# cohensbw/ElPhDynamics

Hardware: AMD Instinct MI355X
Metric: cg_matvecs_per_sec (higher is better)
Workload: dtype f64; 1 GPU; BASELINE config C: Holstein square L=16 Ntau=160 (N=256, Ltau=160, Ndim=40960), un-preconditioned CG iteration, 288 right-hand sides per step on each GPU = 144 independent Markov chain(s) x 2 solve(s) each (2 = the two pseudofermion solves of one HMC force evaluation), 1 GPU(s) with their own chains; nrhs=288, chains_per_gpu=144, ndim=40960, preconditioned=False, form=workgroup-resident: K iterations of the whole batch in one launch (k_cg_wg), parallelism=gpus1xchains144

## Files before the change

elphdynamics_amd/csrc/cg_wg.hip:

```cpp

#include <algorithm>
#include <atomic>
#include <type_traits>

#include "cg_fast_common.h"

#include "cg_wg_dev.h"
#include "pgrid_dev.h"

namespace wg {

#ifdef ELPH_WG_ARRIVE
__device__ unsigned long long g_wg_arrive[4096 * 4];
__device__ unsigned long long g_wg_timeline[4096 * 4];
#define TL(k) do { if (threadIdx.x == 0 && blockIdx.x < 4096) g_wg_timeline[blockIdx.x * 4 + (k)] = (unsigned long long)wall_clock64(); } while (0)
#else
#define TL(k) do { } while (0)
#endif

struct WgRankArgs { CgBufs B; ModelDev m; WgCtl R; ShardCtl Sh; };
template <int NPL, int T, bool SSH, bool UNI, int FORM, bool SHARD, bool X0Z = false, bool RANKS = false>
__global__ void __launch_bounds__(512) k_cg_wg(CgBufs B, ModelDev m, WgCtl R, ShardCtl Sh) {
    static_assert(!RANKS || SHARD, "several ranks per launch: sharded solves only");
    unsigned bid = 0;
// ... 86 lines not shown
            if (lwok) rl[j * HSL + lr + q * LSL] = rg[(size_t)(t0 + j) * N + sc[q]];
            if (X_GLB) {}
            else if (X_REG) xr[X_REG ? j : 0][q] = X0Z ? 0.0 : xg[(size_t)(t0 + j) * N + sc[q]];
            else if (lwok) xl[j * HSL + lr + q * LSL] = X0Z ? 0.0 : xg[(size_t)(t0 + j) * N + sc[q]];
        }
#pragma unroll
    for (int j = 0; j < T + 2; ++j)
#pragma unroll
        for (int q = 0; q < NPL; ++q) {
            p[j][q] = rg[(size_t)wrap(t0 + j - 1) * N + sc[q]];
            if (PH_LDS && (j == 0 || j == T + 1) && lwok) PHALO(j, q) = p[j][q];
        }
#pragma unroll
    for (int j = 0; j < NEJ; ++j)
#pragma unroll
        for (int q = 0; q < NPL; ++q) {
            const double ev = Ech[(size_t)wrap(t0 + j) * m.E_tau_stride + sc[q]];
            if (E_LDS) { if (lwok) el[j * HSL + lr + q * LSL] = ev; }
            else E[E_LDS ? 0 : j][q] = ev;
        }
    unsigned ij[NE];
    Tab<NE, UNI> tab[NT];
    SqCtx<UNI> X;
    SqSsh<NSREG, S_LDS> XS;
    HcCtx XH;
    S8Ctx X8;
    GridCtx XG;
    HgCtx XHG;
    pgrid::Ctx XT;
    if constexpr (GR) {
        XG = grid_ctx(lane, GGX, GGY, m.c_uni, m.s_uni);
        if constexpr (TG) { XT = pgrid::Tri<2, 2>::make_ctx(lane, 2 * GGX, m.c_uni, m.s_uni); XG.k4 = XT.ks; }
    } else if constexpr (HG) {
        XHG = hgrid_ctx<NPL>(lane, HLX, HLY, m.c_uni, m.s_uni);
    } else if constexpr (S8) {
        X8.th = m.s_uni / m.c_uni; X8.k4 = (m.c_uni * m.c_uni) * (m.c_uni * m.c_uni);
        X8.yx = sq_patch_ycross(lane); X8.xodd = (lane >> 1) & 1;
    } else if constexpr (HC) {
        XH.th = m.s_uni / m.c_uni; XH.k3 = m.c_uni * m.c_uni * m.c_uni;
        XH.up = (lane + 16) & (WAVE - 1); XH.dn = (lane + 48) & (WAVE - 1);
    } else if constexpr (SQ && SSH) {
        ssh_chain_select(m, rhs);
        XS.yx = sq_patch_ycross(lane);
        XS.l0 = eall + (size_t)wv * SQ_TABS * WAVE + lane;
#pragma unroll
        for (int j = 0; j <= T; ++j) {
            const double *cj = m.c + (size_t)wrap(t0 + j) * m.cs_tau_stride, *sj = m.s + (size_t)wrap(t0 + j) * m.cs_tau_stride;
            SqTabS tb;
#pragma unroll
            for (int pr = 0; pr < 2; ++pr) {
                const int b0 = m.sq_bond[0 * N + sc[2 * pr]], b2 = m.sq_bond[2 * N + sc[pr]];
                tb.ci[0][pr] = cj[b0]; tb.si[0][pr] = sj[b0];
                tb.ci[1][pr] = cj[b2]; tb.si[1][pr] = sj[b2];
            }
#pragma unroll
            for (int k = 0; k < 4; ++k) {
                const int b1 = m.sq_bond[1 * N + sc[k]], b3 = m.sq_bond[3 * N + sc[k]];
                tb.cx[0][k] = cj[b1]; tb.sx[0][k] = sj[b1];
                tb.cx[1][k] = cj[b3]; tb.sx[1][k] = sj[b3];
            }
            if (S_LDS && j == 0) {
                double *d = eall + (size_t)wv * SQ_TABS * WAVE + lane;
#pragma unroll
                for (int pr = 0; pr < 2; ++pr) {
                    d[(0 + pr) * WAVE] = tb.ci[0][pr]; d[(2 + pr) * WAVE] = tb.si[0][pr];
                    d[(4 + pr) * WAVE] = tb.ci[1][pr]; d[(6 + pr) * WAVE] = tb.si[1][pr];
                }
#pragma unroll
                for (int k = 0; k < 4; ++k) {
                    d[(8 + k) * WAVE] = tb.cx[0][k]; d[(12 + k) * WAVE] = tb.sx[0][k];
                    d[(16 + k) * WAVE] = tb.cx[1][k]; d[(20 + k) * WAVE] = tb.sx[1][k];
                }
            } else {
                XS.t[S_LDS ? (j > 0 ? j - 1 : 0) : (j < NSREG ? j : 0)] = tb;
            }
        }
    } else if constexpr (SQ) {
        X.yx = sq_patch_ycross(lane);
        if constexpr (UNI) {
            X.c[0][0] = m.c_uni; X.s[0][0] = m.s_uni / m.c_uni; X.k4 = (m.c_uni * m.c_uni) * (m.c_uni * m.c_uni);
        } else {
            X.k4 = 1.0;
#pragma unroll
            for (int col = 0; col < 4; ++col)
#pragma unroll
                for (int k = 0; k < 4; ++k) {
                    const int bd = m.sq_bond[col * N + sc[k]];
                    X.c[UNI ? 0 : col][UNI ? 0 : k] = m.c[bd];
                    X.s[UNI ? 0 : col][UNI ? 0 : k] = m.s[bd];
                }
        }
    } else {
#pragma unroll
        for (int e = 0; e < NE; ++e) ij[e] = m.lp_ij[e * WAVE + lane];
        if (SSH) {
            ssh_chain_select(m, rhs);
#pragma unroll
            for (int j = 0; j < NT; ++j)
                load_tab<NE, UNI>(tab[j], m.lp_c + (size_t)wrap(t0 + j) * m.lp_tau_stride, m.lp_s + (size_t)wrap(t0 + j) * m.lp_tau_stride, lane, m);
        } else {
            load_tab<NE, UNI>(tab[0], m.lp_c, m.lp_s, lane, m);
        }
    }
#define EXPV(j, q) (E_LDS ? el[(j) * HSL + lr + (q) * LSL] : E[(SSH || E_LDS) ? 0 : (j)][q])

    constexpr size_t SLOTS_RHS = SLOTS_PER_RHS;
    u64 *const slots0 = R.slots + (size_t)rhs * 2 * SLOTS_RHS;
    u64 *const bnd0 = R.bnd + (size_t)rhs * 2 * G * 2 * HS * 2;
    const int gm = (g == 0) ? G - 1 : g - 1, gp = (g == G - 1) ? 0 : g + 1;
    double rho = S.rho, kmin = S.kmin, eps = S.eps;
    double eps0 = S.eps0, normb = S.normb;

    if (threadIdx.x == 0) { tot[5] = 1.0; if (SHARD) bc[2] = 1.0; }
    if (G > 1) {
        if (wv == 0) {
#pragma unroll
            for (int q = 0; q < NPL; ++q) if (lwok) rhalo[lr + q * LSL] = p[0][q];
        }
        if (wv == W - 1) {
#pragma unroll
            for (int q = 0; q < NPL; ++q) if (lwok) rhalo[HSL + lr + q * LSL] = p[T + 1][q];
        }
    }
    const u64 *gaddr[NPL];
    if constexpr (SHARD) {
#pragma unroll
        for (int q = 0; q < NPL; ++q) {
            const int s = ss[q];
            gaddr[q] = (s < Sh.own_lo) ? sh_ghost(Sh.mail[Sh.rank], 0, L, Sh.cap_ghost, t0, s)
                     : (s >= Sh.own_hi && s < N) ? sh_ghost(Sh.mail[Sh.rank], 1, L, Sh.cap_ghost, t0, s - Sh.own_hi) : nullptr;
        }
        double a0 = 0.0;
#pragma unroll
        for (int q = 0; q < NPL; ++q) if (own[q]) a0 += p[1][q] * p[1][q];
        a0 = wave_sum_dpp(a0);
        if (lane == 0) partA[wv] = a0;
        wg_barrier();
        if (wv == 0) {
            const double mine = wg_sum(partA, W, lane);
            sh_publish<RANKS>(Sh, 0, g, G, mine, 1u, lane);
            const u64 *none[NPL];
#pragma unroll
            for (int q = 0; q < NPL; ++q) none[q] = nullptr;
            double tot = 0.0, dummy[NPL];
            const bool ok = sh_poll<NPL, RANKS>(Sh, true, 0, G, none, 1u, lane, R, tot, dummy);
            if (lane == 0) { bc[0] = tot; if (!ok) bc[2] = 0.0; }
        }
        wg_barrier();
        if (bc[2] == 0.0) return;
        const double bb = bc[0];
        normb = sqrt(bb); eps0 = 1.0; eps = 1.0; rho = bb; kmin = 0.0;
        wg_barrier();
    }
    const double rr_far = (P.tol * normb) * (P.tol * normb) * 1.000001, y_num = 4.0 * (eps0 * normb) * (eps0 * normb);
    const double it_kappa = 0.17 * sqrt(P.kmax);
    STAMP_DECL;
    for (long long seq = 0;; ++seq) {
        const unsigned epoch = R.epoch0 + (unsigned)seq + (SHARD ? 2u : 1u);
        const unsigned par = epoch & 1u;
        u64 *const slotsA = slots0 + (size_t)par * SLOTS_RHS, *const slotsB = slotsA + SLOTS_A;
        u64 *const bnd = bnd0 + (size_t)par * G * 2 * HS * 2;
        const size_t ghp = SHARD ? (size_t)par * 2 * L * Sh.cap_ghost * 2 : 0;
        STAMP(9);
        if (seq == 0) TL(0);
        if (seq == 1) TL(1);
        double (&w)[T + 1][NPL] = zw;
        if constexpr (S8) {
#pragma unroll
            for (int k = 0; k <= T; ++k) w[k][0] = EXPV(k, 0) * p[k][0];
            s8_sweepN<T + 1, false>(w, X8);
#pragma unroll
            for (int k = 0; k <= T; ++k) w[k][0] = p[k + 1][0] - sgn(wrap(t0 + k)) * X8.k4 * w[k][0];
            double gq[T][1];
#pragma unroll
            for (int i = 0; i < T; ++i) gq[i][0] = w[i + 1][0];
            s8_sweepN<T, true>(gq, X8);
#pragma unroll
            for (int i = 0; i < T; ++i) w[i][0] = w[i][0] - sgn(wrap(t0 + i + 1)) * X8.k4 * (EXPV(i + 1, 0) * gq[i][0]);
        } else if constexpr (HC) {
#pragma unroll
            for (int k = 0; k <= T; ++k)
#pragma unroll
                for (int q = 0; q < NPL; ++q) w[k][q] = EXPV(k, q) * ((PH_LDS && k == 0) ? PHALO(0, q) : p[k][q]);
            hc_sweepN<T + 1, false>(w, XH);
#pragma unroll
            for (int k = 0; k <= T; ++k) {
                const double sg = sgn(wrap(t0 + k)) * XH.k3;
#pragma unroll
                for (int q = 0; q < NPL; ++q) w[k][q] = ((PH_LDS && k == T) ? PHALO(1, q) : p[k + 1][q]) - sg * w[k][q];
            }
            auto rev = [&](auto nb, auto j0c) __attribute__((always_inline)) {
                constexpr int NB = decltype(nb)::value, j0 = decltype(j0c)::value;
                double gq[NB][NPL];
#pragma unroll
                for (int i = 0; i < NB; ++i)
#pragma unroll
                    for (int q = 0; q < NPL; ++q) gq[i][q] = w[j0 + i + 1][q];
                hc_sweepN<NB, true>(gq, XH);
#pragma unroll
                for (int i = 0; i < NB; ++i) {
                    const double sg = sgn(wrap(t0 + j0 + i + 1)) * XH.k3;
#pragma unroll
                    for (int q = 0; q < NPL; ++q) w[j0 + i][q] = w[j0 + i][q] - sg * (EXPV(j0 + i + 1, q) * gq[i][q]);
                }
            };
            using std::integral_constant;
            if constexpr (T == 3) { rev(integral_constant<int, 2>(), integral_constant<int, 0>()); rev(integral_constant<int, 1>(), integral_constant<int, 2>()); }
            else rev(integral_constant<int, T>(), integral_constant<int, 0>());
        } else if constexpr (HG) {
#pragma unroll
            for (int k = 0; k <= T; ++k)
#pragma unroll
                for (int q = 0; q < NPL; ++q) w[k][q] = EXPV(k, q) * p[k][q];
            hgrid_sweepN<NPL, T + 1, false>(w, XHG);
#pragma unroll
            for (int k = 0; k <= T; ++k) {
                const double sg = sgn(wrap(t0 + k)) * XHG.k3;
#pragma unroll
                for (int q = 0; q < NPL; ++q) w[k][q] = p[k + 1][q] - sg * w[k][q];
            }
            double gq[T][NPL];
#pragma unroll
            for (int i = 0; i < T; ++i)
#pragma unroll
                for (int q = 0; q < NPL; ++q) gq[i][q] = w[i + 1][q];
            hgrid_sweepN<NPL, T, true>(gq, XHG);
#pragma unroll
            for (int i = 0; i < T; ++i) {
                const double sg = sgn(wrap(t0 + i + 1)) * XHG.k3;
#pragma unroll
                for (int q = 0; q < NPL; ++q) w[i][q] = w[i][q] - sg * (EXPV(i + 1, q) * gq[i][q]);
            }
        } else if constexpr (GR) {
#pragma unroll
            for (int k = 0; k <= T; ++k)
#pragma unroll
                for (int q = 0; q < 4; ++q) w[k][q] = EXPV(k, q) * p[k][q];
            if constexpr (TG) {
#pragma unroll
                for (int k = 0; k <= T; ++k) pgrid::Tri<2, 2>::apply<false>(w[k], XT);
            } else grid_sweepN<T + 1, false, (T >= 4) ? 1 : 2>(w, XG);
#pragma unroll
            for (int k = 0; k <= T; ++k) {
                const double sg = sgn(wrap(t0 + k)) * XG.k4;
#pragma unroll
                for (int q = 0; q < 4; ++q) w[k][q] = p[k + 1][q] - sg * w[k][q];
            }
            constexpr int RBG = (T >= 4) ? 2 : T;
#pragma unroll
            for (int j0 = 0; j0 < T; j0 += RBG) {
                double gq[RBG][4];
#pragma unroll
                for (int i = 0; i < RBG; ++i)
#pragma unroll
                    for (int q = 0; q < 4; ++q) gq[i][q] = w[j0 + i + 1][q];
                if constexpr (TG) {
#pragma unroll
                    for (int i = 0; i < RBG; ++i) pgrid::Tri<2, 2>::apply<true>(gq[i], XT);
                } else grid_sweepN<RBG, true, (T >= 4) ? 1 : 2>(gq, XG);
#pragma unroll
                for (int i = 0; i < RBG; ++i) {
                    const double sg = sgn(wrap(t0 + j0 + i + 1)) * XG.k4;
#pragma unroll
                    for (int q = 0; q < 4; ++q) w[j0 + i][q] = w[j0 + i][q] - sg * (EXPV(j0 + i + 1, q) * gq[i][q]);
                }
            }
        } else if constexpr (SQ) {
#pragma unroll
            for (int k = 0; k <= T; ++k)
#pragma unroll
                for (int q = 0; q < 4; ++q) w[k][q] = EXPV(k, q) * p[k][q];
            if constexpr (SSH) sq_sweepS<T + 1, false, 0>(w, XS);
            else sq_sweepN<T + 1, false, UNI>(w, X);
#pragma unroll
            for (int k = 0; k <= T; ++k) {
                const double sg = UNI ? sgn(wrap(t0 + k)) * X.k4 : sgn(wrap(t0 + k));
#pragma unroll
                for (int q = 0; q < 4; ++q) w[k][q] = p[k + 1][q] - sg * w[k][q];
            }
            constexpr int RB = (T >= 4) ? 2 : T;
#pragma unroll
            for (int j0 = 0; j0 < T; j0 += RB) {
                double gq[RB][4];
#pragma unroll
                for (int i = 0; i < RB; ++i)
#pragma unroll
                    for (int q = 0; q < 4; ++q) gq[i][q] = w[j0 + i + 1][q];
                if constexpr (SSH) sq_sweepS<RB, true, 1>(gq, XS);
                else sq_sweepN<RB, true, UNI>(gq, X);
#pragma unroll
                for (int i = 0; i < RB; ++i) {
                    const double sg = UNI ? sgn(wrap(t0 + j0 + i + 1)) * X.k4 : sgn(wrap(t0 + j0 + i + 1));
#pragma unroll
                    for (int q = 0; q < 4; ++q) w[j0 + i][q] = w[j0 + i][q] - sg * (EXPV(j0 + i + 1, q) * gq[i][q]);
                }
            }
        } else {
#pragma unroll
            for (int k = 0; k <= T; ++k)
#pragma unroll
                for (int q = 0; q < NPL; ++q) slab[k * SL + lane + q * WAVE] = EXPV(k, q) * p[k][q];
            WAVE_LDS_ORDER();
            sweepN<NPL, T + 1, false, UNI, NT, SSH ? 1 : 0, 0>(slab, ij, tab, m.ncol);
#pragma unroll
            for (int k = 0; k <= T; ++k) {
                const double sg = sgn(wrap(t0 + k));
#pragma unroll
                for (int q = 0; q < NPL; ++q) w[k][q] = p[k + 1][q] - sg * slab[k * SL + lane + q * WAVE];
            }
            WAVE_LDS_ORDER();
#pragma unroll
            for (int j = 0; j < T; ++j)
#pragma unroll
                for (int q = 0; q < NPL; ++q) slab[j * SL + lane + q * WAVE] = w[j + 1][q];
            WAVE_LDS_ORDER();
            sweepN<NPL, T, true, UNI, NT, SSH ? 1 : 0, SSH ? 1 : 0>(slab, ij, tab, m.ncol);
#pragma unroll
            for (int j = 0; j < T; ++j) {
                const double sg = sgn(wrap(t0 + j + 1));
#pragma unroll
                for (int q = 0; q < NPL; ++q) w[j][q] = w[j][q] - sg * EXPV(j + 1, q) * slab[j * SL + lane + q * WAVE];
            }
            WAVE_LDS_ORDER();
        }
        double (&z)[T + 1][NPL] = zw;
        int lane_b = lane;
        if constexpr (HC && T >= 3) asm volatile("" : "+v"(lane_b));
        double rr;
        {
        double s_pz = 0.0, s_rz = 0.0, s_zz = 0.0, s_rr = 0.0;
#pragma unroll
        for (int j = 0; j < T; ++j)
#pragma unroll
            for (int q = 0; q < NPL; ++q)
                if (own[q]) {
                    const double rv = rl[j * HSL + lr + q * LSL];
                    s_pz += p[j + 1][q] * z[j][q];
                    s_rz += rv * z[j][q];
                    s_zz += z[j][q] * z[j][q];
                    s_rr += rv * rv;
                }
        {
            const double k4 = wave_sum4(s_pz, s_rz, s_zz, s_rr, lane);
            if (lane < 4) part[lane * 8 + wv] = k4;
        }
        if constexpr (X_GLB) {
#pragma unroll
            for (int j = 0; j < T; ++j)
#pragma unroll
                for (int q = 0; q < NPL; ++q) xr[X_REG ? j : 0][q] = xg[(size_t)(t0 + j) * N + sc[q]];
        }
        if constexpr (SHARD) {
            const int prev = (Sh.rank + Sh.P - 1) % Sh.P, next = (Sh.rank + 1) % Sh.P;
#pragma unroll
            for (int q = 0; q < NPL; ++q) {
                const int s = ss[q];
                const u64 bits = (u64)__double_as_longlong(z[0][q]), tag = (u64)epoch << 32;
                if (s >= Sh.own_lo && s < Sh.own_lo + Sh.n_to_prev) {
                    u64 *d = sh_ghost(Sh.mail[prev], 1, L, Sh.cap_ghost, t0, s - Sh.own_lo) + ghp;
                    st_mail<RANKS>(d, tag | (bits & 0xFFFFFFFFull)); st_mail<RANKS>(d + 1, tag | (bits >> 32));
                }
                if (s >= Sh.own_hi - Sh.n_to_next && s < Sh.own_hi) {
                    u64 *d = sh_ghost(Sh.mail[next], 0, L, Sh.cap_ghost, t0, s - (Sh.own_hi - Sh.n_to_next)) + ghp;
                    st_mail<RANKS>(d, tag | (bits & 0xFFFFFFFFull)); st_mail<RANKS>(d + 1, tag | (bits >> 32));
                }
            }
        }
        if (G > 1) {
            if (wv == 0) {
#pragma unroll
                for (int q = 0; q < NPL; ++q) {
                    st_f64_gran(bnd + (((size_t)g * 2 + 0) * HS + lane_b + q * WAVE) * 2, z[0][q], epoch);
                    if constexpr (HC && T >= 3) __builtin_amdgcn_sched_barrier(0);
                }
            }
            if (wv == W - 1) {
#pragma unroll
                for (int q = 0; q < NPL; ++q) {
                    st_f64_gran(bnd + (((size_t)g * 2 + 1) * HS + lane_b + q * WAVE) * 2, z[T - 1][q], epoch);
                    if constexpr (HC && T >= 3) __builtin_amdgcn_sched_barrier(0);
                }
            }
        }
        STAMP(0);
        wg_barrier();
        STAMP(2);
        double pap, rz, zz, rr0;
        double gz[NPL];
        if constexpr (SHARD) {
            const int rw = (W >= 3) ? 1 : 0;
            u64 *rankrec = Sh.mail[Sh.rank] + (size_t)SH_MAXREC * 2 + (size_t)par * 8 * REC4;
            bool ok = true;
            if (wv == rw) publish_rec4(slotsA, g, sum_part4(part, W, lane), epoch, lane);
            {
                const bool bw = G > 1 && (wv == 0 || wv == W - 1);
                const int th = (wv == 0) ? wrap(t0 - 1) : wrap(t0 + T);
                const u64 *bh = bw ? ((wv == 0) ? bnd + (((size_t)gm * 2 + 1) * HS) * 2 : bnd + (((size_t)gp * 2 + 0) * HS) * 2) : nullptr;
                const u64 *ga2[NPL];
#pragma unroll
                for (int q = 0; q < NPL; ++q) {
                    const int s = ss[q];
                    ga2[q] = !bw ? nullptr
                           : (s < Sh.own_lo) ? sh_ghost(Sh.mail[Sh.rank], 0, L, Sh.cap_ghost, th, s) + ghp
                           : (s >= Sh.own_hi && s < N) ? sh_ghost(Sh.mail[Sh.rank], 1, L, Sh.cap_ghost, th, s - Sh.own_hi) + ghp : nullptr;
                }
                u64 a0[NPL], a1[NPL], h0[NPL], h1[NPL], c0[NPL], c1[NPL];
                long long t_start = 0;
                for (int spin = 0;; ++spin) {
                    bool good = true;
#pragma unroll
                    for (int q = 0; q < NPL; ++q) {
                        if (gaddr[q]) { a0[q] = ld_mail<RANKS>(gaddr[q] + ghp); a1[q] = ld_mail<RANKS>(gaddr[q] + ghp + 1); }
                        if (bh) { h0[q] = ld_gran(bh + 2 * (lane + q * WAVE)); h1[q] = ld_gran(bh + 2 * (lane + q * WAVE) + 1); }
                        if (ga2[q]) { c0[q] = ld_mail<RANKS>(ga2[q]); c1[q] = ld_mail<RANKS>(ga2[q] + 1); }
                    }
#pragma unroll
                    for (int q = 0; q < NPL; ++q) {
                        if (gaddr[q]) good = good && (unsigned)(a0[q] >> 32) == epoch && (unsigned)(a1[q] >> 32) == epoch;
                        if (bh) good = good && (unsigned)(h0[q] >> 32) == epoch && (unsigned)(h1[q] >> 32) == epoch;
                        if (ga2[q]) good = good && (unsigned)(c0[q] >> 32) == epoch && (unsigned)(c1[q] >> 32) == epoch;
                    }
                    if (__all(good)) break;
                    if (poll_bail<NPL>(spin, t_start, lane, R)) { ok = false; break; }
                    __builtin_amdgcn_s_sleep(1);
                }
#pragma unroll
                for (int q = 0; q < NPL; ++q) {
                    gz[q] = gaddr[q] ? __hiloint2double((int)(unsigned)a1[q], (int)(unsigned)a0[q]) : 0.0;
                    if (bw) {
                        const double hv = ga2[q] ? __hiloint2double((int)(unsigned)c1[q], (int)(unsigned)c0[q])
                                                 : __hiloint2double((int)(unsigned)h1[q], (int)(unsigned)h0[q]);
                        zhalo[((wv == 0) ? 0 : HSL) + lr + q * LSL] = hv;
                    }
                }
            }
            if (wv == rw) {
                if (g == 0) {
                    double d0, d1, t4 = 0.0;
                    if (G <= 8) { u64 v[1] = {0}; ok = poll_rec4<1>(slotsA, G, nullptr, nullptr, epoch, lane, R, v, d0, d1) && ok; t4 = sum_rec4<1>(v, G, lane); }
                    else        { u64 v[4] = {0, 0, 0, 0}; ok = poll_rec4<4>(slotsA, G, nullptr, nullptr, epoch, lane, R, v, d0, d1) && ok; t4 = sum_rec4<4>(v, G, lane); }
                    const double mine = __shfl(t4, lane & 6, WAVE);
                    if (lane < 8 * Sh.P) {
                        const u64 bits = (u64)__double_as_longlong(mine);
                        st_mail<RANKS>(Sh.mail[lane >> 3] + (size_t)SH_MAXREC * 2 + (size_t)par * 8 * REC4 + (size_t)Sh.rank * REC4 + (lane & 7),
                               ((u64)epoch << 32) | ((lane & 1) ? (bits >> 32) : (bits & 0xFFFFFFFFull)));
                    }
                }
                u64 v[1] = {0};
                long long t_start = 0;
                for (int spin = 0;; ++spin) {
                    bool good = true;
                    if (lane < REC4 * Sh.P) { v[0] = ld_mail<RANKS>(rankrec + lane); good = (unsigned)(v[0] >> 32) == epoch; }
                    if (__all(good)) break;
                    if (poll_bail<1>(spin, t_start, lane, R)) { ok = false; break; }
                    __builtin_amdgcn_s_sleep(1);
                }
                const double t4 = sum_rec4<1>(v, Sh.P, lane);
                if (lane < 8 && !(lane & 1)) tot[lane >> 1] = t4;
            }
            if (!ok && lane == 0) tot[5] = 0.0;
            wg_barrier();
            if (tot[5] == 0.0) return;
            pap = tot[0]; rz = tot[1]; zz = tot[2]; rr0 = tot[3];
        } else if (G == 1) {
            const double t4 = sum_part4(part, W, lane);
            pap = readlane_f64(t4, 0); rz = readlane_f64(t4, 8); zz = readlane_f64(t4, 16); rr0 = readlane_f64(t4, 24);
        } else {
            constexpr int NSEG = 2 * NPL;
            const int rw = (W > NSEG) ? NSEG : ((W >= 3) ? 1 : 0);
            bool ok = true;
            double t4 = 0.0;
            if (wv == rw) publish_rec4(slotsA, g, sum_part4(part, W, lane), epoch, lane);
            for (int s0 = wv; s0 < NSEG || (s0 == wv && wv == rw); s0 += 2 * W) {
                const int s1 = s0 + W;
                const u64 *b0 = nullptr, *b1 = nullptr;
                if (s0 < NSEG) b0 = bnd + ((((s0 < NPL) ? (size_t)gm * 2 + 1 : (size_t)gp * 2 + 0) * HS) + lane_b + (size_t)(s0 % NPL) * WAVE) * 2;
                if (s1 < NSEG) b1 = bnd + ((((s1 < NPL) ? (size_t)gm * 2 + 1 : (size_t)gp * 2 + 0) * HS) + lane_b + (size_t)(s1 % NPL) * WAVE) * 2;
                const bool recs = (wv == rw && s0 == wv);
                double z0 = 0.0, z1 = 0.0;
                if (G <= 8) {
                    u64 v[1] = {0};
                    ok = poll_rec4<1>(recs ? slotsA : nullptr, G, b0, b1, epoch, lane, R, v, z0, z1) && ok;
                    if (recs) t4 = sum_rec4<1>(v, G, lane);
                } else {
                    u64 v[4] = {0, 0, 0, 0};
                    ok = poll_rec4<4>(recs ? slotsA : nullptr, G, b0, b1, epoch, lane, R, v, z0, z1) && ok;
                    if (recs) t4 = sum_rec4<4>(v, G, lane);
                }
                if (b0 && lwok) zhalo[(size_t)s0 * LSL + lr] = z0;
                if (b1 && lwok) zhalo[(size_t)s1 * LSL + lr] = z1;
                if (!ok) break;
            }
            if (wv == rw && lane < 8 && !(lane & 1)) tot[lane >> 1] = t4;
            if (!ok && lane == 0) tot[5] = 0.0;
#ifdef ELPH_WG_ARRIVE
            if (!ok && lane == 0 && blockIdx.x < 4096) g_wg_arrive[blockIdx.x * 4 + 3] = ((unsigned long long)(seq + 1) << 8) | (1ull << wv);
#endif
            wg_barrier();
            if (tot[5] == 0.0) return;
            pap = tot[0]; rz = tot[1]; zz = tot[2]; rr0 = tot[3];
        }
        STAMP(1);
        rho = rr0;
        const double alpha = rr0 / pap;
        rr = rr0 + alpha * (alpha * zz - 2.0 * rz);
#pragma unroll
        for (int j = 0; j < T; ++j)
#pragma unroll
            for (int q = 0; q < NPL; ++q) {
                const double zq = (SHARD && gaddr[q]) ? gz[q] : z[j][q];
                const double rn = rl[j * HSL + lr + q * LSL] - alpha * zq;
                if (lwok) rl[j * HSL + lr + q * LSL] = rn;
                if (X_GLB) { if (lwok) xg[(size_t)(t0 + j) * N + sc[q]] = xr[X_REG ? j : 0][q] + alpha * p[j + 1][q]; }
                else if (X_REG) xr[X_REG ? j : 0][q] += alpha * p[j + 1][q];
                else if (lwok) xl[j * HSL + lr + q * LSL] += alpha * p[j + 1][q];
            }
        if (G > 1 && (wv == 0 || wv == W - 1)) {
            double *rh = rhalo + ((wv == 0) ? 0 : HSL);
            const double *zh = zhalo + ((wv == 0) ? 0 : HSL);
#pragma unroll
            for (int q = 0; q < NPL; ++q) if (lwok) rh[lr + q * LSL] = rh[lr + q * LSL] - alpha * zh[lr + q * LSL];
        }
        STAMP(3);
        if (!(rr > 1e-3 * rr0)) {
            double a = 0.0;
#pragma unroll
            for (int j = 0; j < T; ++j)
#pragma unroll
                for (int q = 0; q < NPL; ++q) if (own[q]) { const double rn = rl[j * HSL + lr + q * LSL]; a += rn * rn; }
            a = wave_sum_dpp(a);
            if (lane == 0) partF[wv] = a;
            wg_barrier();
            if constexpr (SHARD) {
                if (wv == 0) {
                    sh_publish<RANKS>(Sh, 0, g, G, wg_sum(partF, W, lane), epoch, lane);
                    const u64 *none[NPL];
#pragma unroll
                    for (int q = 0; q < NPL; ++q) none[q] = nullptr;
                    double t = 0.0, dummy[NPL];
                    const bool ok = sh_poll<NPL, RANKS>(Sh, true, 0, G, none, epoch, lane, R, t, dummy);
                    if (lane == 0) { tot[4] = t; if (!ok) tot[5] = 0.0; }
                }
                wg_barrier();
                if (tot[5] == 0.0) return;
                rr = tot[4];
            } else if (G == 1) {
                rr = wg_sum(partF, W, lane);
            } else {
                if (wv == 0) {
                    const double mine = wg_sum(partF, W, lane);
                    if (lane < 2) {
                        const u64 bits = (u64)__double_as_longlong(mine);
                        st_gran(slotsB + 2 * g + lane, ((u64)epoch << 32) | (lane ? (bits >> 32) : (bits & 0xFFFFFFFFull)));
                    }
                    u64 v = 0;
                    const bool ok = poll_records(slotsB, G, epoch, lane, R, v);
                    const int half = (int)(unsigned)v;
                    double t = 0.0;
                    for (int k = 0; k < G; ++k)
                        t += __hiloint2double(__builtin_amdgcn_readlane(half, 2 * k + 1), __builtin_amdgcn_readlane(half, 2 * k));
                    if (lane == 0) { tot[4] = t; if (!ok) tot[5] = 0.0; }
                }
                wg_barrier();
                if (tot[5] == 0.0) return;
                rr = tot[4];
            }
        }
        wg_barrier();
        STAMP(4);
        }
        STAMP(5);
        STAMP(6);
        const long long it = seq + 1;
        const bool fixed = R.fixed_iters > 0;
        int done = 0;
        const bool screened = !P.record_hist && it < (fixed ? R.fixed_iters : P.maxiter) && (fixed || rr > rr_far) &&
                              (rr + rr <= y_num || rr >= y_num + y_num) && (double)it < it_kappa;
        if (!screened) {
            eps = sqrt(rr) / normb;
            const double qq = 2.0 * (double)it / log(2.0 * eps0 / eps);
            const double val = qq * qq;
            kmin = (val > kmin) ? val : kmin;
            if (eps < P.tol) done = 1;
            else if (kmin > P.kmax) done = 2;
            else if (it >= P.maxiter) done = 3;
            if (fixed) done = (it >= R.fixed_iters) ? 3 : 0;
            if (g == 0 && wv == 0 && lane == 0 && P.record_hist) B.hist[(size_t)rhs * P.hist_stride + it] = eps;
        }
        STAMP(7);
        if (done) {
            STAMP_OUT(it);
            TL(2);
            int lane2 = lane;
            asm volatile("" : "+v"(lane2));
#pragma unroll
            for (int j = 0; j < T; ++j)
#pragma unroll
                for (int q = 0; q < NPL; ++q) {
                    const int s2 = SQ ? sq_patch_site(lane2, q) : (HC ? hc_site(lane2, q) : (S8 ? s8_site(lane2) : (GR ? grid_site(lane2, q, GGX, GGY) : (HG ? hgrid_site<NPL>(lane2, q, HLX, HLY) : lane2 + q * WAVE))));
                    if (HC ? hc_real(lane2) : (GR ? lane2 < GGX * GGY : (HG ? lane2 < (HLX / HgDim<NPL>::PX) * (HLY / HgDim<NPL>::PY) : (SQ || s2 < N)))) {
                        if (SHARD) rg[(size_t)(t0 + j) * N + s2] = rl[j * HSL + lr + q * LSL];
                        if (!X_GLB) xg[(size_t)(t0 + j) * N + s2] = X_REG ? xr[X_REG ? j : 0][q] : xl[j * HSL + lr + q * LSL];
                    }
                }
            if (g == 0 && wv == 0 && lane == 0) {
                CgState o = S;
                o.rho = rho; o.kmin = kmin; o.eps = eps; o.seq = it + 1; o.iters = it; o.done = done;
                st2[0] = o;
                st2[1] = o;
            }
            TL(3);
            return;
        }
        const double beta = rr / rho;
        rho = rr;
        {
            const bool lx = (G > 1 && wv == 0), rx = (G > 1 && wv == W - 1);
            const double *sl = rall + ((size_t)((wv > 0) ? wv - 1 : W - 1) * T + (T - 1)) * HSL;
            const double *sr = rall + ((size_t)((wv < W - 1) ? wv + 1 : 0) * T + 0) * HSL;
#pragma unroll
            for (int q = 0; q < NPL; ++q) {
                const double hl = lx ? rhalo[lr + q * LSL] : sl[lr + q * LSL];
                const double hr = rx ? rhalo[HSL + lr + q * LSL] : sr[lr + q * LSL];
                if constexpr (PH_LDS) {
                    const double n0 = hl + beta * PHALO(0, q), n1 = hr + beta * PHALO(1, q);
                    if (lwok) { PHALO(0, q) = n0; PHALO(1, q) = n1; }
                } else {
                    p[0][q] = hl + beta * p[0][q];
                    p[T + 1][q] = hr + beta * p[T + 1][q];
                }
            }
        }
#pragma unroll
        for (int j = 0; j < T; ++j)
#pragma unroll
            for (int q = 0; q < NPL; ++q) p[j + 1][q] = rl[j * HSL + lr + q * LSL] + beta * p[j + 1][q];
        STAMP(8);
    }
#undef EXPV
#undef PHALO
}


struct Shape { int T, W, G; size_t shm; bool sq, hc, s8, gr, hg; int npl; bool tg = false; };

static bool wg_no_dpp() {
    const char *e = getenv("ELPH_WG_NO_DPP");
    return e && e[0] == '1';
}

static bool sq_form(const elph_handle_s *h, const ModelDev &m) {
    return h->shape.dpp() == 2 && m.sq_bond && !wg_no_dpp();
}

static bool hc_form(const elph_handle_s *h, const ModelDev &m) {
    return h->kind == ELPH_MODEL_HOLSTEIN && h->shape.hc12() && m.uniform && !wg_no_dpp();
}

static bool s8_form(const elph_handle_s *h, const ModelDev &m) {
    return h->kind == ELPH_MODEL_HOLSTEIN && h->shape.dpp() == 1 && m.uniform && !wg_no_dpp();
}

static bool gr_form(const elph_handle_s *h, const ModelDev &m, bool for_shard = false) {
    if (h->kind != ELPH_MODEL_HOLSTEIN || !h->shape.small_square() || !m.uniform || m.grid_GX * m.grid_GY < 1 || m.grid_GX * m.grid_GY > 64 || wg_no_dpp()) return false;
    return for_shard || h->shape.dpp() == 0;
}

static bool tg_form(const elph_handle_s *h, const ModelDev &m) {
    return h->kind == ELPH_MODEL_HOLSTEIN && h->shape.kind == LatticeShape::TRIANGULAR && h->shape.GX > 0 && m.uniform && !wg_no_dpp();
}

static int hg_form(const elph_handle_s *h, const ModelDev &m, bool for_shard = false) {
    if (h->kind != ELPH_MODEL_HOLSTEIN || (h->shape.hc12() && !for_shard) || !m.uniform || wg_no_dpp()) return 0;
    return h->shape.hgrid_regs();
}

static int largest_divisor_le8(int n, int cap = 8) { for (int w = std::min(cap, n); w >= 1; --w) if (n % w == 0) return w; return 1; }

static bool pick_shape(const elph_handle_s *h, const ModelDev &m, int forceT, int nrhs, Shape *out) {
    const int L = (int)h->L;
    const bool ssh = (h->kind == ELPH_MODEL_SSH), sq = sq_form(h, m), hc = !sq && hc_form(h, m), s8 = !sq && !hc && s8_form(h, m);
    const bool tg = !sq && !hc && !s8 && tg_form(h, m);
    const bool gr = !sq && !hc && !s8 && (tg || gr_form(h, m));
    const int hgn = (!sq && !hc && !s8 && !gr) ? hg_form(h, m) : 0;
    const bool hg = hgn > 0;
    const int npl = hc ? HC_NPL : (gr ? 4 : (hg ? hgn : h->npl));
    if (h->lp_mc != 4 && !tg) return false;
    if (!hc && !gr && !hg && h->npl > 5) return false;
    bool big_batch = true;
    if (!forceT && L % 2 == 0) {
        const int G2 = (L / 2) / largest_divisor_le8(L / 2);
        big_batch = G2 <= 32 && nrhs > 8 * (32 / G2);
    }
    if (!ssh && !sq && !hc && !gr && !hg && h->npl == 1 && (big_batch || s8)) {
        const int one[3] = {4, 5, 8};
        for (int T : one) {
            if ((forceT && T != forceT) || L % T || L / T > 8 || L / T < 2) continue;
            const int W = L / T;
            const size_t SL = (size_t)npl * WAVE + 2 * WAVE, HS = (size_t)npl * WAVE;
            const size_t shm = ((size_t)W * (s8 ? 0 : T + 1) * SL + 2 * (size_t)W * T * HS + 48 + 4 * HS) * sizeof(double);
            if (shm > 160 * 1024) continue;
            out->T = T; out->W = W; out->G = 1; out->shm = shm; out->sq = false; out->hc = false; out->s8 = s8; out->gr = false; out->hg = false; out->npl = npl;
            return true;
        }
    }
    const int cand[4] = {4, 3, 2, 1};
    for (int T : cand) {
        if (forceT && T != forceT) continue;
        if (T == 3) {
            if (!hc || L % 3 || L % 2) continue;
            if (forceT != 3) {
                const int G2 = (L / 2) / largest_divisor_le8(L / 2), G3 = (L / 3) / largest_divisor_le8(L / 3);
                if (G2 > 32 || G3 > 32) continue;
                const int r2 = 8 * (32 / G2), r3 = 8 * (32 / G3);
                if (nrhs <= r2 || 8.6 * ((nrhs + r3 - 1) / r3) >= 5.7 * ((nrhs + r2 - 1) / r2)) continue;
            }
        }
        if (T == 4) {
            if (!(sq || gr) || !m.uniform || ssh) continue;
            if (forceT != 4) {
                if (L % 2) continue;
                const int G2 = (L / 2) / largest_divisor_le8(L / 2);
                if (G2 > 32 || nrhs <= 8 * (32 / G2)) continue;
            }
        }
        if (gr && T == 3) continue;
        if (hg && T > 2) continue;
        if (T == 2 && (sq || hc || gr || hg) && forceT != 2) {
            const int G1 = L / largest_divisor_le8(L);
            if (G1 <= 32 && L / G1 >= 2 && nrhs <= 8 * (32 / G1)) continue;
        }
        if (T == 2 && !sq && !hc && !gr && !hg && ((ssh && h->npl > 4) || h->npl > 5 || (!ssh && h->npl >= 4 && !m.uniform))) continue;
        if (T == 2 && !sq && !hc && !gr && !hg && (h->npl == 5 || ssh) && forceT != 2) {
            const int G1 = L / largest_divisor_le8(L);
            if (G1 <= 32 && nrhs <= 8 * (32 / G1)) continue;
        }
        if (L % T) continue;
        const int Wt = L / T;
        int W = 0;
        const char *ew = getenv("ELPH_WG_W");
        const int wmax = ew ? std::max(1, atoi(ew)) : 8;
        for (int w = std::min(wmax, Wt); w >= 1; --w) if (Wt % w == 0) { W = w; break; }
        const int G = Wt / W;
        if (G > 32) continue;
        if (G > 1 && W < 2) continue;
        const size_t SL = (size_t)npl * WAVE + 2 * WAVE, HS = (size_t)npl * (hc ? 48 : WAVE);
        const bool s_lds = sq && ssh && T == 2;
        const bool e_lds = ((sq || gr) && T >= 4) || (hc && T >= 2), x_reg = ((sq || gr) && T >= 4) || s_lds || (hc && T >= 3);
        const size_t shm = ((size_t)W * ((sq || hc || s8 || gr || hg) ? 0 : T + 1) * SL + (size_t)(x_reg ? 1 : 2) * W * T * HS +
                            (e_lds ? (hc ? ((size_t)W * T + 1) * HS : (size_t)W * (T + 1) * HS) : 0) + (s_lds ? (size_t)W * wg::SQ_TABS * WAVE : 0) +
                            48 + 4 * HS + ((hc && T >= 3) ? (size_t)W * 2 * HS : 0)) * sizeof(double);
        if (shm > 160 * 1024) continue;
        out->T = T; out->W = W; out->G = G; out->shm = shm; out->sq = sq; out->hc = hc; out->s8 = s8; out->gr = gr; out->hg = hg; out->npl = npl; out->tg = tg;
        return true;
    }
    return false;
}

struct WgCost { const char *form; double a, g, s; const char *measured; };
static const WgCost wg_cost_table[] = {
    {"lane program (FORM 0)",            2.00, 0.12, 0.50, "profiles/r02/time_forms.log: configs B, C, D, E at 1-2 slices per wave; x sites per lane; + 3.9 for SSH at 2 slices, 0.85 T per slice from 4"},
    {"16x16 DPP (FORM 1, Holstein)",     2.66, 0.01, 0.62, "profiles/r03/time_forms.log: 3.5 / 4.0 / 5.2 us at 1 / 2 / 4 slices per wave"},
    {"16x16 DPP, bond phonons",          2.50, 0.00, 1.30, "profiles/r03/time_forms_E_ssh_dpp.log: 3.8 / 5.1 us at 1 / 2 slices"},
    {"honeycomb 12x12 DPP (FORM 2)",     2.10, 0.00, 1.70, "profiles/r03/time_forms_D_honeycomb_dpp.log: 3.8 / 5.5 us at 1 / 2 slices; 8.6 us at 3 (time_forms_D_three_slices_per_wave.log)"},
    {"8x8 DPP (FORM 4), team of one",    2.30, 0.00, 0.00, "profiles/r03/time_wg_B_8x8_dpp_form.log: 2.04-2.3 us whatever the batch"},
    {"GRID (FORM 5)",                    2.90, 0.01, 1.35, "profiles/r04/grid_form_even_L_square_lattices.log: L = 12: 4.3 / 5.6 / 10.0 us at 1 / 2 / 4 slices; L = 14, 10: 3.6-4.0 at 1"},
    {"TGRID (FORM 7, triangular)",       3.20, 0.00, 2.20, "profiles/r04/tgrid_triangular_resident.log: L = 16: 4.9 / 6.7 / 12.4 us at 1 / 2 / 4 slices per wave (4: 69 doubles spilled)"},
    {"HGRID (FORM 6)",                   2.30, 0.01, 1.10, "profiles/r04/hgrid_form_honeycomb_lattices.log: L = 6: 2.5 us (2 registers per lane), L = 10: 3.3-3.8 (4), L = 16: 4.5-5.8 (8); x sites per lane / 4"},
};
static const double wg_streaming_cost[3] = {10.0, 0.56, 0.02};

static double resident_iteration_us(const elph_handle_s *h, const Shape &sh) {
    const bool ssh = h->kind == ELPH_MODEL_SSH;
    if (sh.s8) return wg_cost_table[4].a;
    if (sh.sq && ssh) return wg_cost_table[2].a + wg_cost_table[2].s * sh.T;
    if (sh.hc) return (sh.T == 3) ? 8.6 : wg_cost_table[3].a + wg_cost_table[3].s * sh.T;
    if (sh.sq) return wg_cost_table[1].a + wg_cost_table[1].g * sh.G + wg_cost_table[1].s * sh.T;
    if (sh.gr && sh.tg) return wg_cost_table[6].a + wg_cost_table[6].g * sh.G + wg_cost_table[6].s * sh.T;
    if (sh.gr) return wg_cost_table[5].a + wg_cost_table[5].g * sh.G + wg_cost_table[5].s * sh.T;
    if (sh.hg) return wg_cost_table[7].a + wg_cost_table[7].g * sh.G + wg_cost_table[7].s * sh.T * (sh.npl / 4.0);
    return wg_cost_table[0].a + wg_cost_table[0].g * sh.G + (sh.T >= 4 ? 0.85 : wg_cost_table[0].s) * sh.T * h->npl + ((ssh && sh.T == 2) ? 3.9 : 0.0);
}
static double streaming_iteration_us(const elph_handle_s *h, int nrhs) {
    return wg_streaming_cost[0] + nrhs * (wg_streaming_cost[1] * (double)h->ndim / 40960.0 * (h->kind == ELPH_MODEL_SSH ? 1.1 : 1.0) + wg_streaming_cost[2]);
}

template <int NPL, int T, bool SSH, bool UNI, int FORM, bool SHARD = false, bool X0Z = false>
static hipError_t launch_k(elph_handle_s *h, const Shape &sh, dim3 grid, const CgBufs &B, const ModelDev &m, const WgCtl &R,
                           const ShardCtl &Sh = ShardCtl()) {
// ... 331 lines not shown
```

Baseline: 19.35 million matvec/s.

## Fuse CG residual/solution update with direction update and fold dot products into sweep

For non-sharded kernels with T>=2, the residual and solution updates are moved after the convergence check and merged with the search-direction update into one loop. This saves a separate pass over local memory, and one workgroup barrier per iteration is moved so it sits after the fused update. For the square-patch form, the four dot products are accumulated inside the second stencil sweep instead of in a separate loop. Scalars are made wave-uniform with readfirstlane to keep them in scalar registers. The restructure adds register pressure and changes where the done-path writes x and state. The early-exit path now recomputes the residual on the fly.

```diff
diff --git a/elphdynamics_amd/csrc/cg_wg.hip b/elphdynamics_amd/csrc/cg_wg.hip
--- a/elphdynamics_amd/csrc/cg_wg.hip
+++ b/elphdynamics_amd/csrc/cg_wg.hip
@@ -262,8 +262,13 @@
         normb = sqrt(bb); eps0 = 1.0; eps = 1.0; rho = bb; kmin = 0.0;
         wg_barrier();
     }
-    const double rr_far = (P.tol * normb) * (P.tol * normb) * 1.000001, y_num = 4.0 * (eps0 * normb) * (eps0 * normb);
-    const double it_kappa = 0.17 * sqrt(P.kmax);
+    double rr_far = (P.tol * normb) * (P.tol * normb) * 1.000001, y_num = 4.0 * (eps0 * normb) * (eps0 * normb);
+    double it_kappa = 0.17 * sqrt(P.kmax);
+    constexpr bool FUSED = !SHARD && T >= 2, BSUM = SQ;
+    auto uni = [](double v) __attribute__((always_inline)) {
+        return __hiloint2double(__builtin_amdgcn_readfirstlane(__double2hiint(v)), __builtin_amdgcn_readfirstlane(__double2loint(v)));
+    };
+    if constexpr (FUSED) { rr_far = uni(rr_far); y_num = uni(y_num); it_kappa = uni(it_kappa); normb = uni(normb); eps0 = uni(eps0); }
     STAMP_DECL;
     for (long long seq = 0;; ++seq) {
         const unsigned epoch = R.epoch0 + (unsigned)seq + (SHARD ? 2u : 1u);
@@ -275,6 +280,7 @@
         if (seq == 0) TL(0);
         if (seq == 1) TL(1);
         double (&w)[T + 1][NPL] = zw;
+        double b_pz = 0.0, b_rz = 0.0, b_zz = 0.0, b_rr = 0.0;
         if constexpr (S8) {
 #pragma unroll
             for (int k = 0; k <= T; ++k) w[k][0] = EXPV(k, 0) * p[k][0];
@@ -404,6 +410,19 @@
 #pragma unroll
                     for (int q = 0; q < 4; ++q) w[j0 + i][q] = w[j0 + i][q] - sg * (EXPV(j0 + i + 1, q) * gq[i][q]);
                 }
+                if constexpr (BSUM) {
+#pragma unroll
+                for (int i = 0; i < RB; ++i)
+#pragma unroll
+                    for (int q = 0; q < 4; ++q)
+                        if (own[q]) {
+                            const double rv = rl[(j0 + i) * HSL + lr + q * LSL];
+                            b_pz += p[j0 + i + 1][q] * w[j0 + i][q];
+                            b_rz += rv * w[j0 + i][q];
+                            b_zz += w[j0 + i][q] * w[j0 + i][q];
+                            b_rr += rv * rv;
+                        }
+                }
             }
         } else {
 #pragma unroll
@@ -437,8 +456,10 @@
         int lane_b = lane;
         if constexpr (HC && T >= 3) asm volatile("" : "+v"(lane_b));
         double rr;
+        double alpha_f = 0.0;
         {
-        double s_pz = 0.0, s_rz = 0.0, s_zz = 0.0, s_rr = 0.0;
+        double s_pz = b_pz, s_rz = b_rz, s_zz = b_zz, s_rr = b_rr;
+        if constexpr (!BSUM) {
 #pragma unroll
         for (int j = 0; j < T; ++j)
 #pragma unroll
@@ -450,6 +471,7 @@
                     s_zz += z[j][q] * z[j][q];
                     s_rr += rv * rv;
                 }
+        }
         {
             const double k4 = wave_sum4(s_pz, s_rz, s_zz, s_rr, lane);
             if (lane < 4) part[lane * 8 + wv] = k4;
@@ -612,8 +634,10 @@
         }
         STAMP(1);
         rho = rr0;
-        const double alpha = rr0 / pap;
+        const double alpha = FUSED ? uni(rr0 / pap) : rr0 / pap;
+        if constexpr (FUSED) alpha_f = alpha;
         rr = rr0 + alpha * (alpha * zz - 2.0 * rz);
+        if constexpr (!FUSED) {
 #pragma unroll
         for (int j = 0; j < T; ++j)
 #pragma unroll
@@ -632,12 +656,17 @@
             for (int q = 0; q < NPL; ++q) if (lwok) rh[lr + q * LSL] = rh[lr + q * LSL] - alpha * zh[lr + q * LSL];
         }
         STAMP(3);
+        }
         if (!(rr > 1e-3 * rr0)) {
             double a = 0.0;
 #pragma unroll
             for (int j = 0; j < T; ++j)
 #pragma unroll
-                for (int q = 0; q < NPL; ++q) if (own[q]) { const double rn = rl[j * HSL + lr + q * LSL]; a += rn * rn; }
+                for (int q = 0; q < NPL; ++q)
+                    if (own[q]) {
+                        const double rn = FUSED ? rl[j * HSL + lr + q * LSL] - alpha * z[j][q] : rl[j * HSL + lr + q * LSL];
+                        a += rn * rn;
+                    }
             a = wave_sum_dpp(a);
             if (lane == 0) partF[wv] = a;
             wg_barrier();
@@ -676,8 +705,10 @@
                 rr = tot[4];
             }
         }
-        wg_barrier();
-        STAMP(4);
+        if constexpr (!FUSED) {
+            wg_barrier();
+            STAMP(4);
+        }
         }
         STAMP(5);
         STAMP(6);
@@ -698,11 +729,40 @@
             if (g == 0 && wv == 0 && lane == 0 && P.record_hist) B.hist[(size_t)rhs * P.hist_stride + it] = eps;
         }
         STAMP(7);
+        if constexpr (FUSED) {
+            const double beta = uni(rr / rho);
+#pragma unroll
+            for (int j = 0; j < T; ++j)
+#pragma unroll
+                for (int q = 0; q < NPL; ++q) {
+                    const double rn = rl[j * HSL + lr + q * LSL] - alpha_f * z[j][q];
+                    if (lwok) rl[j * HSL + lr + q * LSL] = rn;
+                    if (X_GLB) { if (lwok) xg[(size_t)(t0 + j) * N + sc[q]] = xr[X_REG ? j : 0][q] + alpha_f * p[j + 1][q]; }
+                    else if (X_REG) xr[X_REG ? j : 0][q] += alpha_f * p[j + 1][q];
+                    else if (lwok) xl[j * HSL + lr + q * LSL] += alpha_f * p[j + 1][q];
+                    if constexpr (!HC) p[j + 1][q] = rn + beta * p[j + 1][q];
+                }
+            if constexpr (HC) {
+                WAVE_LDS_ORDER();
+#pragma unroll
+                for (int j = 0; j < T; ++j)
+#pragma unroll
+                    for (int q = 0; q < NPL; ++q) p[j + 1][q] = rl[j * HSL + lr + q * LSL] + beta * p[j + 1][q];
+            }
+            if (G > 1 && (wv == 0 || wv == W - 1)) {
+                double *rh = rhalo + ((wv == 0) ? 0 : HSL);
+                const double *zh = zhalo + ((wv == 0) ? 0 : HSL);
+#pragma unroll
+                for (int q = 0; q < NPL; ++q) if (lwok) rh[lr + q * LSL] = rh[lr + q * LSL] - alpha_f * zh[lr + q * LSL];
+            }
+            STAMP(3);
+        }
         if (done) {
             STAMP_OUT(it);
             TL(2);
             int lane2 = lane;
             asm volatile("" : "+v"(lane2));
+            const int t0s = FUSED ? (g * W + __builtin_amdgcn_readfirstlane((int)(threadIdx.x >> 6))) * T : t0;
 #pragma unroll
             for (int j = 0; j < T; ++j)
 #pragma unroll
@@ -710,11 +770,11 @@
                     const int s2 = SQ ? sq_patch_site(lane2, q) : (HC ? hc_site(lane2, q) : (S8 ? s8_site(lane2) : (GR ? grid_site(lane2, q, GGX, GGY) : (HG ? hgrid_site<NPL>(lane2, q, HLX, HLY) : lane2 + q * WAVE))));
                     if (HC ? hc_real(lane2) : (GR ? lane2 < GGX * GGY : (HG ? lane2 < (HLX / HgDim<NPL>::PX) * (HLY / HgDim<NPL>::PY) : (SQ || s2 < N)))) {
                         if (SHARD) rg[(size_t)(t0 + j) * N + s2] = rl[j * HSL + lr + q * LSL];
-                        if (!X_GLB) xg[(size_t)(t0 + j) * N + s2] = X_REG ? xr[X_REG ? j : 0][q] : xl[j * HSL + lr + q * LSL];
+                        if (!X_GLB) xg[(size_t)(t0s + j) * N + s2] = X_REG ? xr[X_REG ? j : 0][q] : xl[j * HSL + lr + q * LSL];
                     }
                 }
             if (g == 0 && wv == 0 && lane == 0) {
-                CgState o = S;
+                CgState o = FUSED ? ld_state(st2) : S;
                 o.rho = rho; o.kmin = kmin; o.eps = eps; o.seq = it + 1; o.iters = it; o.done = done;
                 st2[0] = o;
                 st2[1] = o;
@@ -724,6 +784,10 @@
         }
         const double beta = rr / rho;
         rho = rr;
+        if constexpr (FUSED) {
+            wg_barrier();
+            STAMP(4);
+        }
         {
             const bool lx = (G > 1 && wv == 0), rx = (G > 1 && wv == W - 1);
             const double *sl = rall + ((size_t)((wv > 0) ? wv - 1 : W - 1) * T + (T - 1)) * HSL;
@@ -741,10 +805,12 @@
                 }
             }
         }
+        if constexpr (!FUSED) {
 #pragma unroll
         for (int j = 0; j < T; ++j)
 #pragma unroll
             for (int q = 0; q < NPL; ++q) p[j + 1][q] = rl[j * HSL + lr + q * LSL] + beta * p[j + 1][q];
+        }
         STAMP(8);
     }
 #undef EXPV
```

Result: faster. 19.82 million matvec/s (median of 6 runs) (+2.4%).
